# victorkich/ManyTor

Measured on AMD Instinct MI355X. Metric: env-steps/sec (whole node), 1M parallel 4-DoF arms, random actions, higher is better.
Workload: dtype f32

## Files before the change

### manytor_amd/csrc/engine.hip

```cpp
#include <hip/hip_runtime.h>

#include <algorithm>
#include <cmath>
#include <cstdio>
#include <cstdlib>
#include <cstring>
#include <mutex>
#include <new>
#include <iterator>
#include <string>
#include <utility>
#include <vector>

#include "engine_internal.h"
#include "kernels.h"

using namespace mt;

namespace {
thread_local std::string g_last_error;
}

namespace mt {
int fail(mt_handle h, int code, const std::string& msg) {
// ... 42 lines not shown
size_t align_up(size_t v, size_t a) { return (v + a - 1) / a * a; }

int ensure_staging(mt_handle h, size_t bytes) {
  if (h->staging_bytes >= bytes) return MT_OK;
  if (h->staging) {
    MT_HIP(h, hipStreamSynchronize(h->stream));
    MT_HIP(h, hipFree(h->staging));
    h->staging = nullptr;
    h->staging_bytes = 0;
  }
  if (hipMalloc(&h->staging, bytes) != hipSuccess) return fail(h, MT_ERR_ALLOC, "hipMalloc(staging) failed");
  h->staging_bytes = bytes;
  return MT_OK;
}

template <class Tbl>
bool table_matches(const DhConst& t, int dof) {
  if (dof != Tbl::D) return false;
  for (int j = 0; j < dof; ++j)
    if (t.a[j] != Tbl::a(j) || t.d[j] != Tbl::d(j) || t.sa[j] != Tbl::sa(j) || t.ca[j] != Tbl::ca(j) ||
        t.off_deg[j] != Tbl::off(j))
      return false;
  return true;
}

int match_static(const DhConst& t, int dof) {
  if (table_matches<Ref4Table>(t, dof)) return 1;
  if (table_matches<Dh7Table>(t, dof)) return 2;
  return 0;
}

struct BlockCap {
  int64_t from, below;
  int blocks;
};
struct DispatchPolicy {
  int64_t step_split4_max = 49152, step_split2_max = 65536;
  int64_t prefetch_other_max = 131072;
  int64_t fused_split4_max = 32768, fused_split2_max = 131072;
  int64_t reset_split_max = 65536;
  int64_t graph_max = 131072;
  int64_t chains_min = 163840, chains_max = 3145728;
  int64_t chain_split4_max = 16384, chain_split2_max = 49152, chain_prefetch_other_max = 131072;
  int64_t flat_from = 393216;
  BlockCap block_caps[3] = {{147456, 229376, 3}, {229376, 458752, 4}, {458752, 589824, 5}};
  int64_t multi_step_max = 262144;
  int multi_step_k = 5;
  bool fold_reset_into_chains = false;
  int max_recurrence_rotations = 12;
  bool rederive_goals_ref4 = true;
  bool rederive_goals_dh7 = false;
  int rederive_goals_chains = 1;
  int64_t rederive_goals_max_envs = 3145728;
  int64_t ld_pad_above = 16384;
  int ld_pad_floats = 256;
};
static const DispatchPolicy kPolicy{};

static int step_blocks_per_cu(const mt_engine* h, int64_t n_launch) {
  if (h->blocks_per_cu_override >= 0) return h->blocks_per_cu_override;
  if (n_launch >= h->n) return 0;
  for (const BlockCap& c : kPolicy.block_caps)
    if (n_launch >= c.from && n_launch < c.below) return c.blocks;
  return 0;
}
static size_t lds_pad_for_blocks(int blocks_per_cu, size_t static_lds) {
  if (blocks_per_cu <= 0) return 0;
  const size_t per_block = (size_t)163840 / (size_t)blocks_per_cu - 1024;
  return per_block > static_lds ? std::min<size_t>(per_block, 65536) - static_lds : 0;
}

int64_t chain_span(const mt_engine* h, int chains) {
  const int64_t per = (h->n + chains - 1) / chains;
  return (per + 255) / 256 * 256;
}

static bool env_int(const char* name, long long* v) {
  const char* e = std::getenv(name);
  if (!e || !*e) return false;
  *v = std::atoll(e);
  return true;
}

static void choose_dispatch(mt_handle h) {
  const mt_config* cfg = &h->cfg;
  const DispatchPolicy& P = kPolicy;
  const int64_t n = cfg->n_envs;
  long long v = 0;
  h->overrides.clear();
  auto seen = [&](const char* name) { h->overrides += (h->overrides.empty() ? "" : ",") + std::string(name) + "=" + std::to_string(v); };

  h->trig = (cfg->flags & MT_FLAG_HW_TRIG) ? 2 : ((cfg->flags & MT_FLAG_DIRECT_TRIG) ? 1 : 0);
  if (cfg->flags & MT_FLAG_ABLATE_LOOP) h->trig = (cfg->flags & MT_FLAG_ABLATE_OBS) ? 4 : 3;
  else if (cfg->flags & MT_FLAG_ABLATE_OBS) h->trig = 5;
  const bool long_route = h->trig == 0 && (cfg->substeps - 1) / 2 > P.max_recurrence_rotations;
  if (long_route) h->trig = 1;
  h->lds_table = (cfg->flags & MT_FLAG_DH_IN_LDS) != 0 && !long_route;
  h->custom_frames = !(h->args.dh.fo == h->D - 2 && h->args.dh.fe == h->D - 1);
  h->static_kind = ((cfg->flags & (MT_FLAG_NO_SPECIALIZE | MT_FLAG_DH_IN_LDS)) || h->custom_frames) ? 0 : match_static(h->args.dh, h->D);

  int forced_lanes = 0, forced_prefetch = -1;
  if (env_int("MT_SPLIT", &v)) {
    forced_lanes = (v == 2 || v == 4) ? (int)v : 1;
    seen("MT_SPLIT");
  }
  if (env_int("MT_PREFETCH", &v)) {
// ... 38 lines not shown
  if (n < 2 * 256) h->chains = 1;
  h->lazy_chains = true;
  if (env_int("MT_LAZY_CHAINS", &v)) {
    h->lazy_chains = v != 0;
    seen("MT_LAZY_CHAINS");
  }

  h->multi_k = (n <= P.multi_step_max) ? P.multi_step_k : 1;
  if (env_int("MT_ROLLOUT_K", &v)) {
    h->multi_k = (int)std::max<long long>(1, std::min<long long>(64, v));
    seen("MT_ROLLOUT_K");
  }
  h->defer_reset = true;
  if (env_int("MT_DEFER_RESET", &v)) {
    h->defer_reset = v != 0;
    seen("MT_DEFER_RESET");
  }
  h->defer_reset_chained = P.fold_reset_into_chains;
  if (env_int("MT_DEFER_RESET_CHAINS", &v)) {
    h->defer_reset_chained = v != 0;
    seen("MT_DEFER_RESET_CHAINS");
  }
  h->gather_throttle = true;
  if (env_int("MT_GATHER_THROTTLE", &v)) {
    h->gather_throttle = v != 0;
    seen("MT_GATHER_THROTTLE");
  }
  h->snap_in_rollout = true;
  if (env_int("MT_ROLLOUT_SNAP", &v)) {
    h->snap_in_rollout = v != 0;
    seen("MT_ROLLOUT_SNAP");
  }
  h->rollout_early = true;
  if (env_int("MT_ROLLOUT_EARLY", &v)) {
    h->rollout_early = v != 0;
    seen("MT_ROLLOUT_EARLY");
  }

  h->tape_prefetch = false;
  if (env_int("MT_TAPE_PREFETCH", &v)) {
    h->tape_prefetch = v != 0;
    seen("MT_TAPE_PREFETCH");
  }
  h->tape_nt_loads = false;
  if (env_int("MT_TAPE_NT", &v)) {
    h->tape_nt_loads = v != 0;
    seen("MT_TAPE_NT");
  }

  h->ground_compact = true;
  if (env_int("MT_GROUND_COMPACT", &v)) {
    h->ground_compact = v != 0;
    seen("MT_GROUND_COMPACT");
  }

  h->goals_rederive = h->static_kind == 1 ? P.rederive_goals_ref4 : (h->static_kind == 2 ? P.rederive_goals_dh7 : false);
  h->goals_rederive_chains = P.rederive_goals_chains;
  h->goals_rederive_max_envs = P.rederive_goals_max_envs;
  if (env_int("MT_GOALS_REDERIVE", &v)) {
    h->goals_rederive = v != 0 && h->static_kind != 0;
    h->goals_rederive_chains = mt_engine::kMaxChains;
    h->goals_rederive_max_envs = INT64_MAX;
    seen("MT_GOALS_REDERIVE");
  }

  if (h->custom_frames) h->lds_table = false;
  auto schedule_for = [&](int64_t envs, int64_t split4_max, int64_t split2_max, int64_t prefetch_other_max) {
    mt_engine::Schedule s;
    s.step_lanes = envs <= split4_max ? 4 : (envs <= split2_max ? 2 : 1);
    s.prefetch = h->static_kind == 1 || envs <= prefetch_other_max;
    s.rollout_lanes = envs <= P.fused_split4_max ? 4 : (envs <= P.fused_split2_max ? 2 : 1);
    if (forced_lanes) s.step_lanes = s.rollout_lanes = forced_lanes;
    if (forced_prefetch >= 0) s.prefetch = forced_prefetch != 0;
    if (h->custom_frames) s = mt_engine::Schedule{};
    return s;
  };
  h->sched[mt_engine::kBatch] = schedule_for(n, P.step_split4_max, P.step_split2_max, P.prefetch_other_max);
  h->sched[mt_engine::kChain] =
      h->chains > 1 ? schedule_for(chain_span(h, h->chains), P.chain_split4_max, P.chain_split2_max, P.chain_prefetch_other_max)
                    : h->sched[mt_engine::kBatch];
}

#define MT_DISPATCH_D(D_, FN, ...)   \
  switch (D_) {                      \
    case 2: FN<2>(__VA_ARGS__); break; \
    case 3: FN<3>(__VA_ARGS__); break; \
    case 4: FN<4>(__VA_ARGS__); break; \
    case 5: FN<5>(__VA_ARGS__); break; \
    case 6: FN<6>(__VA_ARGS__); break; \
    case 7: FN<7>(__VA_ARGS__); break; \
    case 8: FN<8>(__VA_ARGS__); break; \
    default: break;                  \
  }

struct StepVariant {
  int trig = 0;
  bool lds = false;
  int lanes = 1;
  int pf = 0;
  bool tt = false;
  bool flat = false;
  bool fresh = false;
  bool codes = false;
  bool gc = false;
  int prev = kPrevLoad;
};
// ... 312 lines not shown
void launch_reset_k(mt_handle h, const StepArgs& args) {
  const size_t lds = RANDOM ? (size_t)2 * args.K * kBlock * sizeof(float) : 0;
  if (lds > 65536)
    (void)hipFuncSetAttribute(reinterpret_cast<const void*>(&reset_kernel<D, RANDOM, ONLY_DONE>),
                              hipFuncAttributeMaxDynamicSharedMemorySize, (int)lds);
  hipLaunchKernelGGL((reset_kernel<D, RANDOM, ONLY_DONE>), grid_for(args.n), dim3(kBlock), lds, h->stream, args,
                     h->cfg.radius);
}
template <int D, bool ONLY_DONE>
void launch_reset_split(mt_handle h, const StepArgs& args) {
  constexpr int L = 4;
  const int64_t per_block = kBlock / L;
  const size_t lds = (size_t)2 * args.K * per_block * sizeof(float);
  hipLaunchKernelGGL((reset_split_kernel<D, ONLY_DONE, L>), dim3((unsigned)((args.n + per_block - 1) / per_block)),
                     dim3(kBlock), lds, h->stream, args, h->cfg.radius);
}
template <int D>
void launch_reset_d(mt_handle h, const StepArgs& args, int mode) {
  if (mode == 0) h->codes_valid = false;
  if (mode != 0 && h->reset_split && args.n == h->n)
    return mode == 1 ? launch_reset_split<D, false>(h, args) : launch_reset_split<D, true>(h, args);
  if (mode == 0)
    launch_reset_k<D, false, false>(h, args);
  else if (mode == 1)
    launch_reset_k<D, true, false>(h, args);
  else
    launch_reset_k<D, true, true>(h, args);
}

template <int D>
void launch_observe_d(mt_handle h) {
  hipLaunchKernelGGL((observe_kernel<D>), grid_for(h->n), dim3(kBlock), 0, h->stream, h->args);
}
template <int D>
void launch_check_done_d(mt_handle h) {
  hipLaunchKernelGGL((check_done_kernel<D>), grid_for(h->n), dim3(kBlock), 0, h->stream, h->args);
}
template <int D>
void launch_joints_d(mt_handle h, float* out) {
  hipLaunchKernelGGL((joints_kernel<D>), grid_for(h->n), dim3(kBlock), 0, h->stream, h->args, out);
}

template <class Tbl, int L, int RPF>
void launch_rollout_split_t(mt_handle h, const StepArgs& a, const RolloutArgs& r) {
  const int64_t per_block = kBlock / L;
  const size_t lds = (size_t)3 * h->K * per_block * sizeof(float) + (ActionTrigTable<Tbl>::value ? kTrigEntries * sizeof(SinCos) : 0);
  if (lds > 65536)
    (void)hipFuncSetAttribute(reinterpret_cast<const void*>(&rollout_split_kernel<Tbl, L, RPF>),
                              hipFuncAttributeMaxDynamicSharedMemorySize, (int)lds);
  hipLaunchKernelGGL((rollout_split_kernel<Tbl, L, RPF>), dim3((unsigned)((a.n + per_block - 1) / per_block)), dim3(kBlock), lds,
                     h->stream, a, r);
}

template <class Tbl, int RPF>
void launch_rollout_t(mt_handle h, const StepArgs& a, int lanes, const RolloutArgs& r) {
  if (lanes == 4) return launch_rollout_split_t<Tbl, 4, RPF>(h, a, r);
  if (lanes == 2) return launch_rollout_split_t<Tbl, 2, RPF>(h, a, r);
  const size_t lds = (size_t)3 * h->K * kBlock * sizeof(float) + (ActionTrigTable<Tbl>::value ? kTrigEntries * sizeof(SinCos) : 0);
  if (lds > 65536)
    (void)hipFuncSetAttribute(reinterpret_cast<const void*>(&rollout_kernel<Tbl, RPF>),
                              hipFuncAttributeMaxDynamicSharedMemorySize, (int)lds);
  hipLaunchKernelGGL((rollout_kernel<Tbl, RPF>), grid_for(a.n), dim3(kBlock), lds, h->stream, a, r);
}

template <int D>
void launch_rollout_d(mt_handle h, const StepArgs& a, int lanes, const RolloutArgs& r) {
  launch_rollout_t<RtTable<D>, 0>(h, a, lanes, r);
}
void launch_rollout(mt_handle h, const StepArgs& a, int lanes, const RolloutArgs& r, bool early = false) {
  h->codes_valid = false;
  h->forget_goals();
  if (h->static_kind == 1) return early ? launch_rollout_t<Ref4Table, kPrefetch>(h, a, lanes, r) : launch_rollout_t<Ref4Table, 0>(h, a, lanes, r);
  if (h->static_kind == 2) return early ? launch_rollout_t<Dh7Table, kPrefetch>(h, a, lanes, r) : launch_rollout_t<Dh7Table, 0>(h, a, lanes, r);
  MT_DISPATCH_D(h->D, launch_rollout_d, h, a, lanes, r);
}

template <class Tbl, bool PREFETCH>
void launch_tape_t(mt_handle h, const StepArgs& a, const TapeArgs& r) {
  const size_t lds = (size_t)3 * h->K * kBlock * sizeof(float);
  if (lds > 65536)
    (void)hipFuncSetAttribute(reinterpret_cast<const void*>(&rollout_tape_kernel<Tbl, PREFETCH>),
                              hipFuncAttributeMaxDynamicSharedMemorySize, (int)lds);
  hipLaunchKernelGGL((rollout_tape_kernel<Tbl, PREFETCH>), grid_for(a.n), dim3(kBlock), lds, h->stream, a, r);
}
template <int D>
void launch_tape_d(mt_handle h, const StepArgs& a, const TapeArgs& r) {
  launch_tape_t<RtTable<D>, false>(h, a, r);
}
bool tape_prefetches(const mt_engine* h) { return h->tape_prefetch && h->static_kind != 0; }
void launch_tape(mt_handle h, const StepArgs& a, const TapeArgs& r) {
  const bool pf = tape_prefetches(h);
  if (h->static_kind == 1) return pf ? launch_tape_t<Ref4Table, true>(h, a, r) : launch_tape_t<Ref4Table, false>(h, a, r);
  if (h->static_kind == 2) return pf ? launch_tape_t<Dh7Table, true>(h, a, r) : launch_tape_t<Dh7Table, false>(h, a, r);
  MT_DISPATCH_D(h->D, launch_tape_d, h, a, r);
}

template <class Tbl>
struct TableTag {
  using type = Tbl;
};
template <class F>
void with_table(const mt_engine* h, F&& f) {
  if (h->static_kind == 1) return f(TableTag<Ref4Table>{});
  if (h->static_kind == 2) return f(TableTag<Dh7Table>{});
  switch (h->D) {
    case 2: return f(TableTag<RtTable<2>>{});
    case 3: return f(TableTag<RtTable<3>>{});
    case 4: return f(TableTag<RtTable<4>>{});
    case 5: return f(TableTag<RtTable<5>>{});
    case 6: return f(TableTag<RtTable<6>>{});
    case 7: return f(TableTag<RtTable<7>>{});
    case 8: return f(TableTag<RtTable<8>>{});
    default: return;
  }
}
// ... 501 lines not shown
    h->kernel_name += " [mt_rollout: " + std::to_string(h->chains) + " chains of " + std::to_string(chain_span(h, h->chains)) +
                      " envs, " + (c.v.lanes > 1 ? "L=" + std::to_string(c.v.lanes)
                                                 : "pf=" + std::to_string(c.v.pf) + (c.v.flat ? ", flat=1" : "")) +
                      (c.blocks_per_cu > 0 ? ", " + std::to_string(c.blocks_per_cu) + " blocks/CU" : std::string()) + "]";
  }
  if (h->multi_k > 1 && fusable(h)) {
    const int sp = multi_step_lanes(h);
    h->kernel_name += " [mt_rollout: " + std::to_string(h->multi_k) + " steps per launch, " +
                      (sp > 1 ? "rollout_split_kernel L=" + std::to_string(sp) : std::string("rollout_kernel")) + "]";
  }
  return h->kernel_name.c_str();
}

const char* mt_describe_dispatch(mt_handle h) {
  if (!h) return "";
  const DispatchPolicy& P = kPolicy;
  auto num = [](long long v) { return std::to_string(v); };
  auto b = [](bool v) { return std::string(v ? "true" : "false"); };
  const int64_t span = chain_span(h, h->chains);
  const std::string table = table_name(h);
  const StepPlan sb = batch_plan(h), sc = chain_plan(h);
  const bool multi = h->multi_k > 1 && fusable(h);
  const bool graph = h->graph_mode > 0 || (h->graph_mode < 0 && h->n <= h->graph_max);
  const bool rederive_on = h->goals_rederive && !h->goals_exposed && !h->goals_foreign && !h->points_exposed && !h->trace;
  auto rederives = [&](const StepPlan& p) {
    return rederive_on && p.v.lanes == 1 && p.v.pf != 0 && p.v.tt && (&p == &sb ? h->n : span) <= h->goals_rederive_max_envs;
  };
  std::string caps = "[";
  for (const BlockCap& c : P.block_caps) caps += std::string(caps.size() > 1 ? "," : "") + "[" + num(c.from) + "," + num(c.below) + "," + num(c.blocks) + "]";
  caps += "]";
  std::string& d = h->describe;
  d = "{\"n_envs\":" + num(h->n) + ",\"ld\":" + num(h->ld) + ",\"dof\":" + num(h->D) + ",\"targets\":" + num(h->K) +
      ",\"table\":\"" + table + "\",\"trig\":" + num(h->trig) + ",\"lds_table\":" + b(h->lds_table) + ",\"custom_frames\":" + b(h->custom_frames) +
      ",\"step\":{\"lanes_per_env\":" + num(sb.v.lanes) + ",\"prefetch\":" + b(sb.v.pf != 0) +
      ",\"trig_table\":" + b(sb.v.tt) + ",\"flat\":" + b(sb.v.flat) + "}" +
      ",\"chains\":{\"count\":" + num(h->chains) + ",\"span\":" + num(h->chains > 1 ? span : h->n) + ",\"lazy\":" + b(h->lazy_chains) +
      ",\"lanes_per_env\":" + num(sc.v.lanes) + ",\"prefetch\":" + b(sc.v.pf != 0) + ",\"flat\":" + b(sc.v.flat) +
      ",\"blocks_per_cu\":" + num(h->chains > 1 ? sc.blocks_per_cu : 0) + "}" +
      ",\"rollout\":{\"form\":\"" + (multi ? "multi_step" : (h->chains > 1 ? "chained_steps" : (graph ? "graph_replay" : "launch_per_step"))) +
      "\",\"steps_per_launch\":" + num(multi ? h->multi_k : 1) + ",\"graph\":" + b(!multi && graph) +
      ",\"lanes_per_env\":" + num(multi ? multi_step_lanes(h) : (h->chains > 1 ? sc : sb).v.lanes) +
      ",\"chains\":" + num(multi && !h->chains_forced ? 1 : h->chains) +
      ",\"absorbs_reset\":" + b(h->defer_reset && (multi || chained_rollout_absorbs_reset(h))) + ",\"writes_snapshot\":" + b(h->snap_in_rollout && (multi || (h->chains > 1 && !graph && !h->trace))) + "}" +
      ",\"fused\":{\"usable\":" + b(fusable(h)) + ",\"lanes_per_env\":" + num(h->sched[mt_engine::kBatch].rollout_lanes) + "}" +
      ",\"tape\":{\"usable\":" + b(fusable(h)) + ",\"lanes_per_env\":1,\"chains\":1,\"prefetch\":" + b(tape_prefetches(h)) +
      ",\"nt_loads\":" + b(h->tape_nt_loads) + "}" +
      ",\"shoot\":{\"usable\":" + b(fusable(h)) + ",\"envs_per_block\":" + num(kShootEnvs) + ",\"waves_per_block\":" + num(kShootWaves) + "}" +
      ",\"cem\":{\"usable\":" + b(fusable(h)) + ",\"envs_per_block\":" + num(kShootEnvs) + ",\"waves_per_block\":" + num(kShootWaves) +
      ",\"max_candidates\":64}" +
      ",\"mppi\":{\"usable\":" + b(fusable(h)) + ",\"envs_per_block\":" + num(kShootEnvs) + ",\"waves_per_block\":" + num(kShootWaves) +
      ",\"max_candidates\":64,\"max_steps\":" + num(kMppiMaxSteps) + "}" +
      ",\"policy_rollout\":{\"usable\":" + b(fusable(h)) + ",\"lanes_per_env\":1,\"hidden_extents\":[32,64]}" +
      ",\"reset\":{\"lanes_per_env\":" + num(h->reset_split ? 4 : 1) + "}" +
      ",\"ground_compact\":{\"enabled\":" + b(h->ground_compact) + ",\"step\":" + b(sb.v.gc) + ",\"chains\":" + b(sc.v.gc) + "}" +
      ",\"goals\":{\"rederive\":" + b(!multi && !graph && rederives(h->chains > 1 ? sc : sb)) + ",\"enabled\":" + b(h->goals_rederive) +
      ",\"step\":" + b(rederives(sb)) + ",\"chains\":" + b(rederives(sc)) +
      ",\"chains_rederiving\":" + num(rederives(sc) ? std::min(h->chains, h->goals_rederive_chains) : 0) +
      ",\"launches_rederived\":" + num((long long)h->goals_rederived) + "}" +
      ",\"overrides\":\"" + h->overrides + "\"" +
      ",\"policy\":{\"step_split4_max\":" + num(P.step_split4_max) + ",\"step_split2_max\":" + num(P.step_split2_max) +
      ",\"prefetch_other_max\":" + num(P.prefetch_other_max) + ",\"fused_split4_max\":" + num(P.fused_split4_max) +
      ",\"fused_split2_max\":" + num(P.fused_split2_max) + ",\"reset_split_max\":" + num(P.reset_split_max) +
      ",\"graph_max\":" + num(P.graph_max) + ",\"chains_min\":" + num(P.chains_min) + ",\"chains_max\":" + num(P.chains_max) +
      ",\"chain_split4_max\":" + num(P.chain_split4_max) + ",\"chain_split2_max\":" + num(P.chain_split2_max) +
      ",\"chain_prefetch_other_max\":" + num(P.chain_prefetch_other_max) + ",\"flat_from\":" + num(P.flat_from) +
      ",\"block_caps\":" + caps + ",\"multi_step_max\":" + num(P.multi_step_max) + ",\"multi_step_k\":" + num(P.multi_step_k) +
      ",\"max_recurrence_rotations\":" + num(P.max_recurrence_rotations) + ",\"ld_pad_above\":" + num(P.ld_pad_above) +
      ",\"ld_pad_floats\":" + num(P.ld_pad_floats) + ",\"rederive_goals_ref4\":" + b(P.rederive_goals_ref4) +
      ",\"rederive_goals_dh7\":" + b(P.rederive_goals_dh7) + ",\"rederive_goals_chains\":" + num(P.rederive_goals_chains) +
      ",\"rederive_goals_max_envs\":" + num(P.rederive_goals_max_envs) + "}" +
      ",\"arena_bytes\":" + num((long long)h->arena_bytes) + "}";
  return d.c_str();
}

int mt_set_stream(mt_handle h, void* hip_stream) {
  MT_REQUIRE(nullptr, h != nullptr, "handle is NULL");
  MT_ENTER(h);
  MT_HIP(h, hipStreamSynchronize(h->stream));
  h->stream = (hipStream_t)hip_stream;
  return MT_OK;
}

int mt_use_own_stream(mt_handle h) {
  MT_REQUIRE(nullptr, h != nullptr, "handle is NULL");
  MT_ENTER(h);
  MT_HIP(h, hipStreamSynchronize(h->stream));
  h->stream = h->own_stream;
  return MT_OK;
}

int mt_sync(mt_handle h) {
  MT_REQUIRE(nullptr, h != nullptr, "handle is NULL");
  MT_ENTER_KEEP(h);
  MT_HIP(h, hipStreamSynchronize(h->stream));
  if (h->gather_pending) {
    MT_HIP(h, hipStreamSynchronize(h->side_stream));
    MT_HIP(h, hipEventElapsedTime(&h->last_gather_ms, h->ev_g0, h->ev_g1));
    h->gather_pending = false;
    h->snap_free_known[0] = h->snap_free_known[1] = true;
  }
  return MT_OK;
}

int mt_reset(mt_handle h, const float* points, int layout, int is_device) {
  MT_REQUIRE(nullptr, h != nullptr, "handle is NULL");
  MT_REQUIRE(h, points != nullptr, "points is NULL (use mt_reset_random for device-drawn targets)");
  MT_REQUIRE(h, layout == MT_ENV_MAJOR || layout == MT_SOA, "bad layout");
  if (!is_device && layout == MT_ENV_MAJOR) {
    const int64_t bad = first_unusable(points, h->n * 3 * h->K, kMaxFiniteBits);
    if (bad >= 0) return fail(h, MT_ERR_INVALID_ARG, "mt_reset: points element " + std::to_string(bad) + " is NaN or infinite");
  }
  if (!is_device && layout == MT_SOA)
    for (int r = 0; r < 3 * h->K; ++r) {
      const int64_t bad = first_unusable(points + (int64_t)r * h->ld, h->n, kMaxFiniteBits);
      if (bad >= 0)
        return fail(h, MT_ERR_INVALID_ARG, "mt_reset: points row " + std::to_string(r) + " element " + std::to_string(bad) + " is NaN or infinite");
    }
  MT_ENTER(h);
  const int rows = 3 * h->K;
  if (layout == MT_SOA) {
    const size_t bytes = (size_t)rows * h->ld * 4;
    MT_HIP(h, hipMemcpyAsync(h->args.points, points, bytes, is_device ? hipMemcpyDeviceToDevice : hipMemcpyHostToDevice,
                             h->stream));
// ... 1980 lines not shown
```

### manytor_amd/csrc/engine_internal.h

```cpp
#pragma once
#include <hip/hip_runtime.h>

#include <cstdlib>
#include <string>
#include <vector>

#include "step_args.h"

struct mt_comm;

struct mt_engine {
  static constexpr int kMaxChains = 4;
  mt_config cfg{};
  int64_t n = 0, ld = 0;
  int D = 0, K = 0;
  hipStream_t own_stream = nullptr;
  hipStream_t stream = nullptr;
  hipEvent_t ev0 = nullptr, ev1 = nullptr;
  hipEvent_t ev1c[kMaxChains] = {nullptr, nullptr, nullptr, nullptr};
  int timer_ends = 0;
  bool timer_with_gather = false;
  struct LapRec {
    uint32_t begin, n_begin, end0, n_end;
  };
// ... 33 lines not shown
    uint64_t seed = 0;
  };
  GoalsRow goals_row[kMaxChains];
  void forget_goals() {
    for (GoalsRow& g : goals_row) g = GoalsRow{};
  }
  void goals_are(GoalsRow::Kind kind, uint64_t seed = 0, uint32_t step = 0) {
    for (GoalsRow& g : goals_row) g = GoalsRow{kind, step, seed};
  }
  bool goals_rederive = true;
  int goals_rederive_chains = kMaxChains;
  int64_t goals_rederive_max_envs = INT64_MAX;
  bool goals_foreign = false;
  uint64_t goals_rederived = 0;
  bool trig_steps = false;
  int static_kind = 0;
  mt_comm* comm = nullptr;
  hipStream_t side_stream = nullptr;
  hipEvent_t ev_snap = nullptr, ev_g0 = nullptr, ev_g1 = nullptr;
  float* snap = nullptr;
  hipEvent_t ev_gdone[2] = {nullptr, nullptr};
  bool snap_free_known[2] = {true, true};
  int snap_next = 0;
  bool gather_throttle = true;
  float* snap_row(int p) const { return snap + (size_t)p * (size_t)n; }
  void* reduce_scratch = nullptr;
  size_t reduce_scratch_bytes = 0;
  bool reset_split = false;
  struct RolloutGraph {
    int T;
    int chains;
    mt::StepArgs args;
    hipGraphExec_t exec[kMaxChains];
  };
  std::vector<RolloutGraph> graphs;
  std::vector<int> graph_seen;
  uint32_t* graph_step0 = nullptr;
  int graph_mode = -1;
  int64_t graph_max = 131072;
  int chains = 1;
  bool chains_forced = false;
  int multi_k = 1;
  bool rollout_early = true;
  bool defer_reset_chained = false;
  bool defer_reset = true;
  bool reset_pending = false;
  uint64_t pend_seed = 0;
  uint32_t pend_episode = 0;
  bool snap_in_rollout = true;
  bool snap_valid = false;
  bool tape_prefetch = false;
  bool tape_nt_loads = false;
  bool ground_compact = true;
  std::string overrides;
  std::string describe;
  hipStream_t chain_streams[kMaxChains] = {nullptr, nullptr, nullptr, nullptr};
  hipEvent_t ev_fork = nullptr, ev_join[kMaxChains] = {nullptr, nullptr, nullptr, nullptr};
  bool forked = false;
  bool lazy_chains = true;
  bool gather_pending = false;
  bool gather_inplace = false;
  float last_gather_ms = 0.f;
  int cu_count = 0;
  std::string err;
  std::string kernel_name;
};

namespace mt {

inline unsigned event_flags(bool timing) {
  static const bool fenced = [] {
    const char* e = std::getenv("MT_EVENT_FENCE");
    return e && *e && std::atoi(e) != 0;
  }();
  return (timing ? 0u : (unsigned)hipEventDisableTiming) | (fenced ? 0u : (unsigned)hipEventDisableSystemFence);
}

int fail(mt_handle h, int code, const std::string& msg);

class DeviceGuard {
 public:
  explicit DeviceGuard(int device) {
    if (hipGetDevice(&prev_) != hipSuccess) prev_ = -1;
    err_ = (prev_ == device) ? hipSuccess : hipSetDevice(device);
    changed_ = (err_ == hipSuccess && prev_ != device);
  }
  ~DeviceGuard() {
    if (changed_ && prev_ >= 0) (void)hipSetDevice(prev_);
  }
  hipError_t error() const { return err_; }

 private:
  int prev_ = -1;
  hipError_t err_ = hipSuccess;
  bool changed_ = false;
};

inline dim3 grid_for(int64_t n) { return dim3((unsigned)((n + kBlock - 1) / kBlock)); }

inline bool snapshot_trusted(mt_engine* h) {
  if (h->stream != h->own_stream) return false;
  hipStreamCaptureStatus st = hipStreamCaptureStatusNone;
  if (hipStreamIsCapturing(h->stream, &st) != hipSuccess) {
    (void)hipGetLastError();
    return false;
  }
// ... 66 lines not shown
```

### manytor_amd/csrc/kernels.h

```cpp
#pragma once
#include <hip/hip_runtime.h>
#include <stdint.h>

#include <type_traits>

#include "mt_math.h"
#include "philox.h"
#include "step_args.h"

namespace mt {

#ifndef MT_NT_STORES
#define MT_NT_STORES 1
#endif
template <typename T>
using global_ptr = __attribute__((address_space(1))) T*;

__device__ __forceinline__ global_ptr<char> uniform_row(const void* row) {
  const uint64_t v = reinterpret_cast<uint64_t>(row);
  const uint32_t lo = __builtin_amdgcn_readfirstlane((uint32_t)v);
  const uint32_t hi = __builtin_amdgcn_readfirstlane((uint32_t)(v >> 32));
  return (global_ptr<char>)(((uint64_t)hi << 32) | lo);
}
#ifndef MT_PLAIN_LANE_OFFSET
// ... 634 lines not shown
      cache->c[j] = c[j];
    }
    cache->zmin = fminf(el[2], e[2]);
  }
  zmin = fminf(zmin, fminf(el[2], e[2]));
  return zmin;
}

template <class Tbl, int TRIG, bool CACHED = false, bool TABLE = false>
__device__ __forceinline__ float route_kinematics(const Tbl& t, int S, float inv_sm1, const float (&g)[Tbl::D],
                                                  const float (&act)[Tbl::D], float (&el)[3], float (&e)[3],
                                                  PoseCache<Tbl::D>* cache = nullptr, bool cache_valid = false,
                                                  const SinCos* trig = nullptr, bool prev_whole = false) {
  if constexpr (TRIG <= 2) {
    if (__builtin_expect(__any(wide_route<Tbl, TABLE>(g, act, prev_whole)), 0))
      return route_kinematics_wide<Tbl, CACHED>(t, S, g, act, el, e, cache);
  }
  return route_kinematics_narrow<Tbl, TRIG, CACHED, TABLE>(t, S, inv_sm1, g, act, el, e, cache, cache_valid, trig, prev_whole);
}

template <class Tbl>
struct GroundQueue {
  static constexpr int kJoints = ZJoints<Tbl>::value - 1;
  static constexpr int kFields = 6 * kJoints;
  static constexpr int kCap = (14336 / (4 * kFields) >= kBlock / 2) ? kBlock / 2 : (14336 / (4 * kFields)) / 32 * 32;
  static_assert(kCap >= 32 && 2 * kCap <= kBlock, "one half route per lane");
  uint32_t count;
  float zres[2 * kCap];
  float field[kFields][kCap];
};

template <class Tbl>
__device__ __forceinline__ float half_route_zmin(const Tbl& t, float (&s)[Tbl::D], float (&c)[Tbl::D], const float (&sd)[Tbl::D],
                                                 const float (&cd)[Tbl::D], int n_half, int mine) {
  constexpr int D = Tbl::D;
  constexpr int JN = ZJoints<Tbl>::value;
  float zm = 3.0e38f, zo, ze;
#pragma unroll 2
  for (int it = 1; it <= n_half; ++it) {
    rotate_pose<D, JN, +1>(s, c, sd, cd);
    chain_z<Tbl>(s, c, t, zo, ze);
    if (it <= mine) zm = fminf(zm, fminf(zo, ze));
  }
  return zm;
}

struct NoGroundQueue {
  uint32_t count;
};
__device__ __forceinline__ void ground_queue_reset(uint32_t* count) {
  if (threadIdx.x == 0) *count = 0u;
}

template <class Tbl, bool TABLE>
__device__ __forceinline__ float route_kinematics_block(const Tbl& t, int S, float inv_sm1, const float (&g)[Tbl::D],
                                                        const float (&act)[Tbl::D], float (&el)[3], float (&e)[3],
                                                        const SinCos* trig, bool prev_whole, bool live, GroundQueue<Tbl>& q) {
  constexpr int D = Tbl::D;
  constexpr int JN = ZJoints<Tbl>::value;
  constexpr int kCap = GroundQueue<Tbl>::kCap;
  const int nf = (S - 1) / 2;
  const int nb = S - 2 - nf;
  float zmin;
  bool undecided = false;
  float sF[D], cF[D], sA[D], cA[D], sd[D], cd[D];
  if (__builtin_expect(__any(live && wide_route<Tbl, TABLE>(g, act, prev_whole)), 0)) {
    zmin = route_kinematics_wide<Tbl, false>(t, S, g, act, el, e, nullptr);
  } else {
    float st[D];
#pragma unroll
    for (int j = 0; j < D; ++j) st[j] = (act[j] - g[j]) * inv_sm1;
    float p[D][3], zo, ze;
    action_sincos<Tbl, TABLE>(t, act, sA, cA, trig);
    chain_all<Tbl>(sA, cA, t, p);
    pick_frames<Tbl>(t, p, el, e);
    zmin = fminf(el[2], e[2]);
#pragma unroll
    for (int j = 0; j < D; ++j) {
      sF[j] = 0.f;
      cF[j] = 1.f;
    }
    prev_pose_sincos<Tbl, TABLE>(t, g, sF, cF, trig, prev_whole);
    chain_z<Tbl>(sF, cF, t, zo, ze);
    zmin = fminf(zmin, fminf(zo, ze));
    sincos_increment<D, JN>(st, sd, cd);
    sA[0] = 0.f;
    cA[0] = 1.f;
    undecided = live && !(zmin < 0.f);
  }

  const unsigned long long um = __ballot(undecided);
  uint32_t slot = kCap;
  if (um != 0ull) {
    uint32_t base = 0u;
    if ((threadIdx.x & 63u) == 0u) base = atomicAdd(&q.count, (uint32_t)__popcll(um));
    base = (uint32_t)__builtin_amdgcn_readfirstlane((int)base);
    slot = base + __builtin_amdgcn_mbcnt_hi((uint32_t)(um >> 32), __builtin_amdgcn_mbcnt_lo((uint32_t)um, 0u));
  }
  const bool queued = undecided && slot < (uint32_t)kCap;
  if (queued) {
#pragma unroll
    for (int j = 1; j < JN; ++j) {
      float(*f)[kCap] = q.field + 6 * (j - 1);
      f[0][slot] = sF[j];
      f[1][slot] = cF[j];
      f[2][slot] = sA[j];
      f[3][slot] = cA[j];
      f[4][slot] = sd[j];
      f[5][slot] = cd[j];
    }
  }
  if (undecided && !queued) {
    zmin = fminf(zmin, half_route_zmin<Tbl>(t, sF, cF, sd, cd, nf, nf));
#pragma unroll
    for (int j = 1; j < JN; ++j) sd[j] = -sd[j];
    zmin = fminf(zmin, half_route_zmin<Tbl>(t, sA, cA, sd, cd, nf, nb));
  }
  __syncthreads();

  const uint32_t routes = q.count < (uint32_t)kCap ? q.count : (uint32_t)kCap;
  const uint32_t w = (threadIdx.x + 64u * (blockIdx.x & 3u)) & (uint32_t)(kBlock - 1);
  if (w < 2u * routes) {
    const uint32_t r = w >> 1;
    const bool backward = (w & 1u) != 0u;
    float sW[D], cW[D], sdW[D], cdW[D];
#pragma unroll
    for (int j = 0; j < D; ++j) {
      sW[j] = 0.f;
      cW[j] = 1.f;
      sdW[j] = 0.f;
      cdW[j] = 1.f;
    }
#pragma unroll
    for (int j = 1; j < JN; ++j) {
      const float(*f)[kCap] = q.field + 6 * (j - 1);
      sW[j] = backward ? f[2][r] : f[0][r];
      cW[j] = backward ? f[3][r] : f[1][r];
      const float sdj = f[4][r];
      sdW[j] = backward ? -sdj : sdj;
      cdW[j] = f[5][r];
    }
    q.zres[w] = half_route_zmin<Tbl>(t, sW, cW, sdW, cdW, nf, backward ? nb : nf);
  }
  __syncthreads();
  if (queued) zmin = fminf(zmin, fminf(q.zres[2u * slot], q.zres[2u * slot + 1u]));
  return zmin;
}

__device__ __forceinline__ void record_finished(const StepArgs& a, uint32_t i, uint32_t episode, float ret) {
  LaneOffset<true> o4{i * 4u};
  str(a.last_return, o4, ret);
  if (a.ring_slots)
    a.ring[(int64_t)((episode - a.episode0) % a.ring_slots) * a.ld + i] = ret;
}

#ifdef MT_STAMPS
#define MT_STAMP(a, i, slot)                                                                 \
  do {                                                                                       \
    __builtin_amdgcn_sched_barrier(0);                                                       \
    unsigned long long t__;                                                                  \
    asm volatile("s_memtime %0\n\ts_waitcnt lgkmcnt(0)" : "=s"(t__)::"memory");              \
    __builtin_amdgcn_sched_barrier(0);                                                       \
    if ((a).stamps && (threadIdx.x & 63) == 0) (a).stamps[(size_t)((i) >> 6) * 8 + (slot)] = t__; \
  } while (0)
#else
#define MT_STAMP(a, i, slot) \
  do {                       \
  } while (0)
#endif

__device__ __forceinline__ bool unusable_angle(float v) { return (__float_as_uint(v) & 0x7FFFFFFFu) > 0x47000000u; }

template <class Tbl, int TRIG>
constexpr int step_min_waves() { return (TRIG == 0 && Tbl::D >= 6 && Tbl::D <= 7) ? 8 : 1; }

constexpr int kPrefetch = 8;

__device__ __forceinline__ void draw_targets_wave(uint64_t seed, uint64_t env0, uint32_t episode, bool need, int K, float radius,
                                                  float* col0, uint8_t* slots);

enum : int { kPrevLoad = 0, kPrevZero = 1, kPrevDraw = 2 };
template <class Tbl, bool SAMPLE, int TRIG, bool LDS, int PF = 0, bool TT = false, bool FLAT = false, bool FRESH = false,
          bool CODES = false, bool GC = false, int PREV = kPrevLoad>
__global__ __launch_bounds__(kBlock, (PF ? 1 : step_min_waves<Tbl, TRIG>())) void step_kernel(const StepArgs a) {
  constexpr int D = Tbl::D;
  static_assert(PREV == kPrevLoad || CODES, "the previous pose is re-derived by the code-reading kernels (the HBM-bound launches)");
  static_assert(!GC || (TRIG == 0 && !LDS && !FRESH), "the block-cooperative ground test serves the recurrence");
  static_assert(!TT || (SAMPLE && TRIG == 0 && !LDS && ActionTrigTable<Tbl>::value), "the table serves sampled actions of a static table");
  static_assert(!FRESH || TT, "the reset prologue exists for the sampled-action kernels of the static tables");
  static_assert(!CODES || (PF && TT && !FRESH), "codes are read by the prefetch kernels of the static tables");
  extern __shared__ float fresh_stage[];
  __shared__ uint8_t fresh_slots[FRESH ? kBlock / 64 : 1][64];
  __shared__ DhConst sh;
  __shared__ __attribute__((aligned(16))) SinCos trig_lds[TT ? kTrigEntries : 1];
  __shared__ std::conditional_t<GC, GroundQueue<Tbl>, NoGroundQueue> ground_q;
  float4 trig_v;
  if (TT) trig_v = trig_table_load(a.trig_table);
  if constexpr (GC) {
    ground_queue_reset(&ground_q.count);
// ... 695 lines not shown
  draw_targets_split<L>(seed, env_id, episode, go, K, radius, q, e, put);
  __builtin_amdgcn_wave_barrier();
  if (live && go)
    for (int k = (int)q; k < K; k += L) store_target(a, ld, i, k, staged_code(col + 2 * k * EPB, EPB), radius);
  if (live && q == 0) {
    if (ONLY_DONE && dn == 2) a.done[i] = 0;
    if (go) {
      float s[D], c[D], p[D][3];
#pragma unroll
      for (int j = 0; j < D; ++j) {
        (a.goals + j * ld)[i] = 0.f;
        sincos_deg(a.dh.off_deg[j], s[j], c[j]);
      }
      const RtTableF<D> t{a.dh};
      chain_all<RtTableF<D>>(s, c, t, p);
      float el0[3], e0[3];
      pick_frames<RtTableF<D>>(t, p, el0, e0);
#pragma unroll
      for (int qq = 0; qq < 3; ++qq) (a.ee + qq * ld)[i] = e0[qq];
      if (ONLY_DONE)
        record_finished(a, i, old_episode, old_total);
      else
        a.last_return[i] = old_total;
      a.total_reward[i] = 0.f;
      a.reward[i] = 0;
      a.done[i] = 0;
      a.alive[i] = all_alive_mask(K);
      a.episodes[i] = episode;
    }
  }
  if (lane == 0) a.done_bits[first >> 6] = 0ull;
}

template <int STRIDE>
struct TargetColumn {
  float* col;
  __device__ __forceinline__ float& row(int r) const { return col[r * STRIDE]; }
  __device__ __forceinline__ float& cell(int k, int c) const { return row(3 * k + c); }
  __device__ __forceinline__ float* target(int k) const { return col + 3 * k * STRIDE; }
  __device__ __forceinline__ void get(int k, float& x, float& y, float& z) const { x = target(k)[0], y = target(k)[STRIDE], z = target(k)[2 * STRIDE]; }
  __device__ __forceinline__ void put(int k, float x, float y, float z) const { target(k)[0] = x, target(k)[STRIDE] = y, target(k)[2 * STRIDE] = z; }
  __device__ __forceinline__ void zero(int k) const { put(k, 0.f, 0.f, 0.f); }
};

struct RolloutArgs {
  int32_t T;
  uint32_t step0;
  uint32_t auto_reset;
  float radius;
  uint32_t reset_first, reset_episode, reset_seed_lo, reset_seed_hi;
  float* snap;
};

template <class Tbl, int RPF = 0>
__global__ __launch_bounds__(kBlock) void rollout_kernel(const StepArgs a, const RolloutArgs r) {
  extern __shared__ __attribute__((aligned(16))) float tile[];
  constexpr int D = Tbl::D;
  constexpr bool kTable = ActionTrigTable<Tbl>::value;
  const Tbl t = TableMaker<Tbl>::make(a.dh);
  const SinCos* trig = nullptr;
  float4 trig_v;
  if constexpr (kTable) {
    trig = reinterpret_cast<const SinCos*>(tile + 3 * a.K * kBlock);
    trig_v = trig_table_load(a.trig_table);
    if (!RPF) trig_table_commit(reinterpret_cast<SinCos*>(tile + 3 * a.K * kBlock), trig_v);
  }
  const uint32_t i = blockIdx.x * kBlock + threadIdx.x;
  LaneOffset<true> o4{i * 4u}, o1{i};
  const bool stay = (kTable && RPF) || r.reset_first != 0;
  if (!stay && i >= a.n) return;
  const int64_t ld = a.ld;
  const uint64_t seed = ((uint64_t)a.seed_hi << 32) | a.seed_lo;
  const uint64_t env_id = (uint64_t)(a.env_base + i);
  const TargetColumn<kBlock> tc{tile + threadIdx.x};
  __shared__ uint8_t draw_slots[kBlock / 64][64];

  const uint32_t all_alive = all_alive_mask(a.K);
  const bool fresh = r.reset_first != 0;
  float g[D];
#pragma unroll
  for (int j = 0; j < D; ++j) g[j] = fresh ? 0.f : ldr(a.goals + j * ld, o4);
  uint32_t am = fresh ? all_alive : ldr(a.alive, o4);
  float total = ldr(a.total_reward, o4);
  uint32_t episode = fresh ? r.reset_episode : (r.auto_reset ? ldr(a.episodes, o4) : 0u);
  bool ended = fresh, dirty = fresh;
  float tx[RPF ? RPF : 1][3];
  if (fresh) {
    const bool mine = i < a.n;
    if (mine) str(a.last_return, o4, total);
    total = 0.f;
    const uint32_t lane = threadIdx.x & 63u;
    draw_targets_wave(((uint64_t)r.reset_seed_hi << 32) | r.reset_seed_lo, (uint64_t)(a.env_base + (i - lane)), episode, mine, a.K, r.radius,
                      tile + (threadIdx.x - lane), draw_slots[threadIdx.x >> 6]);
    decode_column(tc.col, a.K, r.radius);
    if (!(kTable && RPF) && !mine) return;
  } else if (RPF) {
#pragma unroll
    for (int k = 0; k < RPF; ++k)
      if (k < a.K) {
#pragma unroll
        for (int q = 0; q < 3; ++q) tx[k][q] = ldr(a.points + (int64_t)(3 * k + q) * ld, o4);
      }
  } else {
    for (int k = 0; k < 3 * a.K; ++k) tc.row(k) = ldr(a.points + (int64_t)k * ld, o4);
  }
  PoseCache<D> pose;
  bool pose_valid = false;

  auto finish_step = [&](const float (&act)[D], const float (&el)[3], const float (&e)[3], float zmin) {
    const bool ground = zmin < 0.f;
    if (a.zmin) str_stream(a.zmin, o4, zmin);

    uint32_t nam = am;
    for (int k = 0; k < a.K; ++k) {
      float x, y, z, dist = 0.f, rr = 0.f, th = 0.f;
      tc.get(k, x, y, z);
      if ((am >> k) & 1u) {
        observe_target(el, x, y, z, dist, rr, th);
        if (within_box(e, x, y, z, a.tol)) nam &= ~(1u << k);
      } else if ((x != 0.f) | (y != 0.f) | (z != 0.f)) {
        tc.zero(k);
        dirty = true;
      }
      float* orow = a.obs + (int64_t)(3 * k) * ld;
      str_stream(orow, o4, dist);
      str_stream(orow + ld, o4, rr);
      str_stream(orow + 2 * ld, o4, th);
    }
    const int32_t rew = ground ? -1 : ((nam != am) ? 1 : 0);
    bool done = (nam == 0u);
    if (a.flags & MT_FLAG_TERMINATE_ON_GROUND) done |= ground;
    total += (float)rew;
    am = nam;
#pragma unroll
    for (int j = 0; j < D; ++j) g[j] = act[j];
#pragma unroll
    for (int q = 0; q < 3; ++q) str_stream(a.ee + q * ld, o4, e[q]);
    str_stream(a.reward, o4, rew);
    str_stream(a.done, o1, (uint8_t)(done ? (r.auto_reset ? 2 : 1) : 0));
    const unsigned long long bits = __ballot(done);
    if ((threadIdx.x & 63) == 0) a.done_bits[i >> 6] = bits;

    if (done && r.auto_reset) {
      record_finished(a, i, episode, total);
      ended = true;
      total = 0.f;
      am = all_alive;
      episode += 1u;
#pragma unroll
      for (int j = 0; j < D; ++j) g[j] = 0.f;
      pose_valid = false;
      draw_targets(seed, env_id, episode, a.K, r.radius, [&](int k, float x, float y, float z) { tc.put(k, x, y, z); });
      dirty = true;
    }
  };

  int s = 0;
  if (RPF) {
    float act[D], el[3], e[3];
    draw_action<D>(seed, env_id, r.step0, act);
    if constexpr (kTable) {
      complete_before_here(act);
      trig_table_commit(reinterpret_cast<SinCos*>(tile + 3 * a.K * kBlock), trig_v);
      if (i >= a.n) return;
    }
    const float zmin = route_kinematics<Tbl, 0, true, kTable>(t, a.S, a.inv_sm1, g, act, el, e, &pose, false, trig,
                                                              (a.flags & kFlagWholeGoals) != 0);
    pose_valid = true;
    if (!fresh) {
#pragma unroll
      for (int k = 0; k < RPF; ++k)
        if (k < a.K) {
#pragma unroll
          for (int q = 0; q < 3; ++q) tc.cell(k, q) = tx[k][q];
        }
      for (int k = 3 * RPF; k < 3 * a.K; ++k) tc.row(k) = ldr(a.points + (int64_t)k * ld, o4);
    }
    finish_step(act, el, e, zmin);
    s = 1;
  }
  for (; s < r.T; ++s) {
    float act[D], el[3], e[3];
    draw_action<D>(seed, env_id, r.step0 + (uint32_t)s, act);
    const float zmin = route_kinematics<Tbl, 0, true, kTable>(t, a.S, a.inv_sm1, g, act, el, e, &pose, pose_valid, trig,
                                                              (a.flags & kFlagWholeGoals) != 0 || s > 0);
    pose_valid = true;
    finish_step(act, el, e, zmin);
  }

#pragma unroll
  for (int j = 0; j < D; ++j) str(a.goals + j * ld, o4, g[j]);
  str(a.alive, o4, am);
  str(a.total_reward, o4, total);
  if (r.snap) str(r.snap, o4, total);
  if (ended) str(a.episodes, o4, episode);
  if (dirty)
    for (int k = 0; k < 3 * a.K; ++k) str(a.points + (int64_t)k * ld, o4, tc.row(k));
}

template <class Tbl, int L, int RPF = 0>
__global__ __launch_bounds__(kBlock) void rollout_split_kernel(const StepArgs a, const RolloutArgs r) {
  static_assert(L == 2 || L == 4, "an env is spread over 2 or 4 lanes");
  extern __shared__ __attribute__((aligned(16))) float tile[];
  constexpr int D = Tbl::D;
  constexpr int EPW = 64 / L;
  constexpr int EPB = kBlock / L;
  constexpr int PFS = (RPF + L - 1) / L;
  constexpr bool kTable = ActionTrigTable<Tbl>::value;
  const Tbl t = TableMaker<Tbl>::make(a.dh);
  const SinCos* trig = nullptr;
  float4 trig_v;
  if constexpr (kTable) {
    trig = reinterpret_cast<const SinCos*>(tile + 3 * a.K * EPB);
    trig_v = trig_table_load(a.trig_table);
    if (!RPF) trig_table_commit(reinterpret_cast<SinCos*>(tile + 3 * a.K * EPB), trig_v);
  }
  const uint32_t lane = threadIdx.x & 63u;
  const uint32_t wave = blockIdx.x * (kBlock / 64) + (threadIdx.x >> 6);
  const uint32_t q = lane / EPW;
  const int64_t first = (int64_t)wave * EPW;
  if (first >= a.n) {
    if constexpr (kTable) {
      if (RPF) trig_table_commit(reinterpret_cast<SinCos*>(tile + 3 * a.K * EPB), trig_v);
    }
    return;
  }
  const uint32_t env = (uint32_t)first + lane % EPW;
  const bool live = env < a.n;
  const uint32_t i = live ? env : (uint32_t)(a.n - 1);
  const int64_t ld = a.ld;
  const uint64_t seed = ((uint64_t)a.seed_hi << 32) | a.seed_lo;
  const uint64_t env_id = (uint64_t)(a.env_base + i);
  const TargetColumn<EPB> tc{tile + (threadIdx.x >> 6) * EPW + lane % EPW};
  const bool backward = (q & 1u) != 0;

  const uint32_t all_alive = all_alive_mask(a.K);
  const bool fresh = r.reset_first != 0;
  float g[D];
#pragma unroll
  for (int j = 0; j < D; ++j) g[j] = fresh ? 0.f : (a.goals + j * ld)[i];
  uint32_t am = fresh ? all_alive : a.alive[i];
  float total = a.total_reward[i];
// ... 1859 lines not shown
```

Measured before the change: 33.13 billion.

## Add block-level ground-compaction queue to the single-lane fused rollout kernel

Adds a GC template variant of rollout_kernel that routes the ground-contact refinement through a shared block queue. Undecided envs are compacted and their interpolated ground checks are spread across the whole block instead of running divergently per thread. Pose caching is kept, and two alternating counters avoid an extra barrier for the queue reset. The variant is used when the rollout runs with one lane per env and at least 262144 envs. The cost is block-wide syncs every step, extra LDS for the queue, and out-of-range threads that must stay alive through the rollout.

```diff
diff --git a/manytor_amd/csrc/engine.hip b/manytor_amd/csrc/engine.hip
--- a/manytor_amd/csrc/engine.hip
+++ b/manytor_amd/csrc/engine.hip
@@ -118,6 +118,7 @@
   bool rederive_goals_dh7 = false;
   int rederive_goals_chains = 1;
   int64_t rederive_goals_max_envs = 3145728;
+  int64_t rollout_gc_min_envs = 262144;
   int64_t ld_pad_above = 16384;
   int ld_pad_floats = 256;
 };
@@ -262,6 +263,11 @@
   if (env_int("MT_GROUND_COMPACT", &v)) {
     h->ground_compact = v != 0;
     seen("MT_GROUND_COMPACT");
+  }
+  h->rollout_gc_min_envs = P.rollout_gc_min_envs;
+  if (env_int("MT_ROLLOUT_GC_MIN", &v)) {
+    h->rollout_gc_min_envs = std::max<long long>(0, v);
+    seen("MT_ROLLOUT_GC_MIN");
   }
 
   h->goals_rederive = h->static_kind == 1 ? P.rederive_goals_ref4 : (h->static_kind == 2 ? P.rederive_goals_dh7 : false);
@@ -680,15 +686,32 @@
                      h->stream, a, r);
 }
 
+static bool rollout_compacts(const mt_engine* h, int64_t n_launch, int lanes) {
+  return lanes == 1 && ground_compacts(h, true) && n_launch >= h->rollout_gc_min_envs;
+}
+
+template <class Tbl, int RPF, bool GC>
+void launch_rollout_k(mt_handle h, const StepArgs& a, const RolloutArgs& r) {
+  const size_t lds = (size_t)3 * h->K * kBlock * sizeof(float) + (ActionTrigTable<Tbl>::value ? kTrigEntries * sizeof(SinCos) : 0);
+  if (lds + (GC ? ground_queue_bytes(h) : 0) > 65536)
+    (void)hipFuncSetAttribute(reinterpret_cast<const void*>(&rollout_kernel<Tbl, RPF, GC>),
+                              hipFuncAttributeMaxDynamicSharedMemorySize, (int)lds);
+  hipLaunchKernelGGL((rollout_kernel<Tbl, RPF, GC>), grid_for(a.n), dim3(kBlock), lds, h->stream, a, r);
+}
 template <class Tbl, int RPF>
 void launch_rollout_t(mt_handle h, const StepArgs& a, int lanes, const RolloutArgs& r) {
   if (lanes == 4) return launch_rollout_split_t<Tbl, 4, RPF>(h, a, r);
   if (lanes == 2) return launch_rollout_split_t<Tbl, 2, RPF>(h, a, r);
-  const size_t lds = (size_t)3 * h->K * kBlock * sizeof(float) + (ActionTrigTable<Tbl>::value ? kTrigEntries * sizeof(SinCos) : 0);
-  if (lds > 65536)
-    (void)hipFuncSetAttribute(reinterpret_cast<const void*>(&rollout_kernel<Tbl, RPF>),
-                              hipFuncAttributeMaxDynamicSharedMemorySize, (int)lds);
-  hipLaunchKernelGGL((rollout_kernel<Tbl, RPF>), grid_for(a.n), dim3(kBlock), lds, h->stream, a, r);
+  if constexpr (Tbl::D <= 5) {
+    if (rollout_compacts(h, a.n, lanes)) {
+      if (a.n < 1 || (int64_t)grid_for(a.n).x * kBlock > a.ld) {
+        std::fprintf(stderr, "manytor: a ground-compacting rollout launch of %lld envs over rows of %lld\n", (long long)a.n, (long long)a.ld);
+        std::abort();
+      }
+      return launch_rollout_k<Tbl, RPF, true>(h, a, r);
+    }
+  }
+  launch_rollout_k<Tbl, RPF, false>(h, a, r);
 }
 
 template <int D>
@@ -1296,7 +1319,10 @@
       ",\"max_candidates\":64,\"max_steps\":" + num(kMppiMaxSteps) + "}" +
       ",\"policy_rollout\":{\"usable\":" + b(fusable(h)) + ",\"lanes_per_env\":1,\"hidden_extents\":[32,64]}" +
       ",\"reset\":{\"lanes_per_env\":" + num(h->reset_split ? 4 : 1) + "}" +
-      ",\"ground_compact\":{\"enabled\":" + b(h->ground_compact) + ",\"step\":" + b(sb.v.gc) + ",\"chains\":" + b(sc.v.gc) + "}" +
+      ",\"ground_compact\":{\"enabled\":" + b(h->ground_compact) + ",\"step\":" + b(sb.v.gc) + ",\"chains\":" + b(sc.v.gc) +
+      ",\"fused\":" + b(fusable(h) && rollout_compacts(h, h->n, h->sched[mt_engine::kBatch].rollout_lanes)) +
+      ",\"multi_step\":" + b(multi && rollout_compacts(h, (h->chains > 1 && h->chains_forced) ? span : h->n, multi_step_lanes(h))) +
+      ",\"rollout_min_envs\":" + num(h->rollout_gc_min_envs) + "}" +
       ",\"goals\":{\"rederive\":" + b(!multi && !graph && rederives(h->chains > 1 ? sc : sb)) + ",\"enabled\":" + b(h->goals_rederive) +
       ",\"step\":" + b(rederives(sb)) + ",\"chains\":" + b(rederives(sc)) +
       ",\"chains_rederiving\":" + num(rederives(sc) ? std::min(h->chains, h->goals_rederive_chains) : 0) +
@@ -1312,7 +1338,7 @@
       ",\"max_recurrence_rotations\":" + num(P.max_recurrence_rotations) + ",\"ld_pad_above\":" + num(P.ld_pad_above) +
       ",\"ld_pad_floats\":" + num(P.ld_pad_floats) + ",\"rederive_goals_ref4\":" + b(P.rederive_goals_ref4) +
       ",\"rederive_goals_dh7\":" + b(P.rederive_goals_dh7) + ",\"rederive_goals_chains\":" + num(P.rederive_goals_chains) +
-      ",\"rederive_goals_max_envs\":" + num(P.rederive_goals_max_envs) + "}" +
+      ",\"rederive_goals_max_envs\":" + num(P.rederive_goals_max_envs) + ",\"rollout_gc_min_envs\":" + num(P.rollout_gc_min_envs) + "}" +
       ",\"arena_bytes\":" + num((long long)h->arena_bytes) + "}";
   return d.c_str();
 }
diff --git a/manytor_amd/csrc/engine_internal.h b/manytor_amd/csrc/engine_internal.h
--- a/manytor_amd/csrc/engine_internal.h
+++ b/manytor_amd/csrc/engine_internal.h
@@ -109,6 +109,7 @@
   bool tape_prefetch = false;
   bool tape_nt_loads = false;
   bool ground_compact = true;
+  int64_t rollout_gc_min_envs = INT64_MAX;
   std::string overrides;
   std::string describe;
   hipStream_t chain_streams[kMaxChains] = {nullptr, nullptr, nullptr, nullptr};
diff --git a/manytor_amd/csrc/kernels.h b/manytor_amd/csrc/kernels.h
--- a/manytor_amd/csrc/kernels.h
+++ b/manytor_amd/csrc/kernels.h
@@ -710,10 +710,12 @@
   if (threadIdx.x == 0) *count = 0u;
 }
 
-template <class Tbl, bool TABLE>
-__device__ __forceinline__ float route_kinematics_block(const Tbl& t, int S, float inv_sm1, const float (&g)[Tbl::D],
-                                                        const float (&act)[Tbl::D], float (&el)[3], float (&e)[3],
-                                                        const SinCos* trig, bool prev_whole, bool live, GroundQueue<Tbl>& q) {
+template <class Tbl, bool TABLE, bool CACHED>
+__device__ __forceinline__ float route_kinematics_block_impl(const Tbl& t, int S, float inv_sm1, const float (&g)[Tbl::D],
+                                                             const float (&act)[Tbl::D], float (&el)[3], float (&e)[3],
+                                                             const SinCos* trig, bool prev_whole, bool live, GroundQueue<Tbl>& q,
+                                                             uint32_t* count, uint32_t* next_count, PoseCache<Tbl::D>* cache,
+                                                             bool cache_valid) {
   constexpr int D = Tbl::D;
   constexpr int JN = ZJoints<Tbl>::value;
   constexpr int kCap = GroundQueue<Tbl>::kCap;
@@ -723,7 +725,44 @@
   bool undecided = false;
   float sF[D], cF[D], sA[D], cA[D], sd[D], cd[D];
   if (__builtin_expect(__any(live && wide_route<Tbl, TABLE>(g, act, prev_whole)), 0)) {
-    zmin = route_kinematics_wide<Tbl, false>(t, S, g, act, el, e, nullptr);
+    zmin = route_kinematics_wide<Tbl, CACHED>(t, S, g, act, el, e, cache);
+  } else if constexpr (CACHED) {
+    const bool use_cache = __all(cache_valid || !live);
+    float st[D];
+#pragma unroll
+    for (int j = 0; j < D; ++j) st[j] = (act[j] - g[j]) * inv_sm1;
+    float p[D][3], zo, ze;
+    action_sincos<Tbl, TABLE>(t, act, sA, cA, trig);
+    chain_all<Tbl>(sA, cA, t, p);
+    pick_frames<Tbl>(t, p, el, e);
+    zmin = fminf(el[2], e[2]);
+#pragma unroll
+    for (int j = 0; j < D; ++j) {
+      sF[j] = 0.f;
+      cF[j] = 1.f;
+    }
+    if (use_cache) {
+#pragma unroll
+      for (int j = 1; j < JN; ++j) {
+        sF[j] = cache->s[j];
+        cF[j] = cache->c[j];
+      }
+      zmin = fminf(zmin, cache->zmin);
+    } else {
+      prev_pose_sincos<Tbl, TABLE>(t, g, sF, cF, trig, prev_whole);
+      chain_z<Tbl>(sF, cF, t, zo, ze);
+      zmin = fminf(zmin, fminf(zo, ze));
+    }
+#pragma unroll
+    for (int j = 1; j < JN; ++j) {
+      cache->s[j] = sA[j];
+      cache->c[j] = cA[j];
+    }
+    cache->zmin = fminf(el[2], e[2]);
+    sincos_increment<D, JN>(st, sd, cd);
+    sA[0] = 0.f;
+    cA[0] = 1.f;
+    undecided = live && !(zmin < 0.f);
   } else {
     float st[D];
 #pragma unroll
@@ -751,7 +790,7 @@
   uint32_t slot = kCap;
   if (um != 0ull) {
     uint32_t base = 0u;
-    if ((threadIdx.x & 63u) == 0u) base = atomicAdd(&q.count, (uint32_t)__popcll(um));
+    if ((threadIdx.x & 63u) == 0u) base = atomicAdd(count, (uint32_t)__popcll(um));
     base = (uint32_t)__builtin_amdgcn_readfirstlane((int)base);
     slot = base + __builtin_amdgcn_mbcnt_hi((uint32_t)(um >> 32), __builtin_amdgcn_mbcnt_lo((uint32_t)um, 0u));
   }
@@ -776,7 +815,9 @@
   }
   __syncthreads();
 
-  const uint32_t routes = q.count < (uint32_t)kCap ? q.count : (uint32_t)kCap;
+  const uint32_t queued_routes = *count;
+  const uint32_t routes = queued_routes < (uint32_t)kCap ? queued_routes : (uint32_t)kCap;
+  if constexpr (CACHED) ground_queue_reset(next_count);
   const uint32_t w = (threadIdx.x + 64u * (blockIdx.x & 3u)) & (uint32_t)(kBlock - 1);
   if (w < 2u * routes) {
     const uint32_t r = w >> 1;
@@ -803,6 +844,13 @@
   __syncthreads();
   if (queued) zmin = fminf(zmin, fminf(q.zres[2u * slot], q.zres[2u * slot + 1u]));
   return zmin;
+}
+template <class Tbl, bool TABLE>
+__device__ __forceinline__ float route_kinematics_block(const Tbl& t, int S, float inv_sm1, const float (&g)[Tbl::D],
+                                                        const float (&act)[Tbl::D], float (&el)[3], float (&e)[3],
+                                                        const SinCos* trig, bool prev_whole, bool live, GroundQueue<Tbl>& q) {
+  return route_kinematics_block_impl<Tbl, TABLE, false>(t, S, inv_sm1, g, act, el, e, trig, prev_whole, live, q, &q.count, nullptr,
+                                                        nullptr, false);
 }
 
 __device__ __forceinline__ void record_finished(const StepArgs& a, uint32_t i, uint32_t episode, float ret) {
@@ -1604,12 +1652,18 @@
   float* snap;
 };
 
-template <class Tbl, int RPF = 0>
+template <class Tbl, int RPF = 0, bool GC = false>
 __global__ __launch_bounds__(kBlock) void rollout_kernel(const StepArgs a, const RolloutArgs r) {
   extern __shared__ __attribute__((aligned(16))) float tile[];
   constexpr int D = Tbl::D;
   constexpr bool kTable = ActionTrigTable<Tbl>::value;
   const Tbl t = TableMaker<Tbl>::make(a.dh);
+  __shared__ std::conditional_t<GC, GroundQueue<Tbl>, NoGroundQueue> ground_q;
+  __shared__ uint32_t ground_count_odd;
+  if constexpr (GC) {
+    ground_queue_reset(&ground_q.count);
+    if (!kTable) __syncthreads();
+  }
   const SinCos* trig = nullptr;
   float4 trig_v;
   if constexpr (kTable) {
@@ -1617,9 +1671,11 @@
     trig_v = trig_table_load(a.trig_table);
     if (!RPF) trig_table_commit(reinterpret_cast<SinCos*>(tile + 3 * a.K * kBlock), trig_v);
   }
-  const uint32_t i = blockIdx.x * kBlock + threadIdx.x;
+  const uint32_t slot_i = blockIdx.x * kBlock + threadIdx.x;
+  const bool live = !GC || slot_i < a.n;
+  const uint32_t i = live ? slot_i : (uint32_t)(a.n - 1);
   LaneOffset<true> o4{i * 4u}, o1{i};
-  const bool stay = (kTable && RPF) || r.reset_first != 0;
+  const bool stay = GC || (kTable && RPF) || r.reset_first != 0;
   if (!stay && i >= a.n) return;
   const int64_t ld = a.ld;
   const uint64_t seed = ((uint64_t)a.seed_hi << 32) | a.seed_lo;
@@ -1638,14 +1694,14 @@
   bool ended = fresh, dirty = fresh;
   float tx[RPF ? RPF : 1][3];
   if (fresh) {
-    const bool mine = i < a.n;
+    const bool mine = slot_i < a.n;
     if (mine) str(a.last_return, o4, total);
     total = 0.f;
     const uint32_t lane = threadIdx.x & 63u;
-    draw_targets_wave(((uint64_t)r.reset_seed_hi << 32) | r.reset_seed_lo, (uint64_t)(a.env_base + (i - lane)), episode, mine, a.K, r.radius,
+    draw_targets_wave(((uint64_t)r.reset_seed_hi << 32) | r.reset_seed_lo, (uint64_t)(a.env_base + (slot_i - lane)), episode, mine, a.K, r.radius,
                       tile + (threadIdx.x - lane), draw_slots[threadIdx.x >> 6]);
     decode_column(tc.col, a.K, r.radius);
-    if (!(kTable && RPF) && !mine) return;
+    if (!GC && !(kTable && RPF) && !mine) return;
   } else if (RPF) {
 #pragma unroll
     for (int k = 0; k < RPF; ++k)
@@ -1707,6 +1763,20 @@
     }
   };
 
+  auto kinematics = [&](const float (&act)[D], float (&el)[3], float (&e)[3], int step, bool prev_whole) {
+    float zmin;
+    if constexpr (GC) {
+      uint32_t* const even = &ground_q.count;
+      uint32_t* const odd = &ground_count_odd;
+      zmin = route_kinematics_block_impl<Tbl, kTable, true>(t, a.S, a.inv_sm1, g, act, el, e, trig, prev_whole, live, ground_q,
+                                                            (step & 1) ? odd : even, (step & 1) ? even : odd, &pose, pose_valid);
+    } else {
+      zmin = route_kinematics<Tbl, 0, true, kTable>(t, a.S, a.inv_sm1, g, act, el, e, &pose, pose_valid, trig, prev_whole);
+    }
+    pose_valid = true;
+    return zmin;
+  };
+
   int s = 0;
   if (RPF) {
     float act[D], el[3], e[3];
@@ -1714,11 +1784,9 @@
     if constexpr (kTable) {
       complete_before_here(act);
       trig_table_commit(reinterpret_cast<SinCos*>(tile + 3 * a.K * kBlock), trig_v);
-      if (i >= a.n) return;
-    }
-    const float zmin = route_kinematics<Tbl, 0, true, kTable>(t, a.S, a.inv_sm1, g, act, el, e, &pose, false, trig,
-                                                              (a.flags & kFlagWholeGoals) != 0);
-    pose_valid = true;
+      if (!GC && i >= a.n) return;
+    }
+    const float zmin = kinematics(act, el, e, 0, (a.flags & kFlagWholeGoals) != 0);
     if (!fresh) {
 #pragma unroll
       for (int k = 0; k < RPF; ++k)
@@ -1728,18 +1796,17 @@
         }
       for (int k = 3 * RPF; k < 3 * a.K; ++k) tc.row(k) = ldr(a.points + (int64_t)k * ld, o4);
     }
-    finish_step(act, el, e, zmin);
+    if (live) finish_step(act, el, e, zmin);
     s = 1;
   }
   for (; s < r.T; ++s) {
     float act[D], el[3], e[3];
     draw_action<D>(seed, env_id, r.step0 + (uint32_t)s, act);
-    const float zmin = route_kinematics<Tbl, 0, true, kTable>(t, a.S, a.inv_sm1, g, act, el, e, &pose, pose_valid, trig,
-                                                              (a.flags & kFlagWholeGoals) != 0 || s > 0);
-    pose_valid = true;
-    finish_step(act, el, e, zmin);
-  }
-
+    const float zmin = kinematics(act, el, e, s, (a.flags & kFlagWholeGoals) != 0 || s > 0);
+    if (live) finish_step(act, el, e, zmin);
+  }
+
+  if (!live) return;
 #pragma unroll
   for (int j = 0; j < D; ++j) str(a.goals + j * ld, o4, g[j]);
   str(a.alive, o4, am);
```

Result: no change. 33.14 billion, median of 2 (+0.0%).
